# b-tudor/mpmcxx

Hardware: AMD Instinct MI355X
Metric: energy-evals/sec (10k-atom LJ+Ewald+polar box); 1/2/4/8-GPU scaling (higher is better)
Workload: dtype f64

## Files before the change

mpmcxx_amd/csrc/context.cpp:

```cpp
#include "context.h"

using namespace mpmc;

thread_local std::string mpmc::g_create_error;

extern "C" int mpmc_abi_version(void) { return MPMC_ABI_VERSION; }

extern "C" int mpmc_device_count(int *count) {
	int n = 0;
	hipError_t e = hipGetDeviceCount(&n);
	if (count) *count = (e == hipSuccess) ? n : 0;
	return (e == hipSuccess) ? MPMC_OK : MPMC_ERR_NO_DEVICE;
}

extern "C" int mpmc_device_synchronize(int device) {
	if (hipSetDevice(device) != hipSuccess) return MPMC_ERR_NO_DEVICE;
	return hipDeviceSynchronize() == hipSuccess ? MPMC_OK : MPMC_ERR_HIP;
}
extern "C" int mpmc_device_name(int device, char *name, int capacity) {
	if (!name || capacity < 1) return MPMC_ERR_ARG;
	name[0] = 0;
	hipDeviceProp_t prop;
	if (hipGetDeviceProperties(&prop, device) != hipSuccess) return MPMC_ERR_NO_DEVICE;
	std::snprintf(name, (size_t)capacity, "%s (%s, %d CUs)", prop.name, prop.gcnArchName, prop.multiProcessorCount);
// ... 1292 lines not shown
		if (v < -1 || v > 1) return MPMC_ERR_ARG;
		t.stream_mode = v;
	} else if (k == "pair_kernel") {
		if (v < 0 || v > 2) return MPMC_ERR_ARG;
		t.pair_kernel = v;
	} else if (k == "pair_waves") {
		if (v != 0 && v != 1 && v != 4) return MPMC_ERR_ARG;
		t.pair_waves = v;
	} else if (k == "fast_geometry") t.fast_geometry = on;
	else if (k == "dense_symmetric") t.dense_symmetric = on;
	else if (k == "sort_grid") {
		if (v < -1 || v > 0) return MPMC_ERR_ARG;
		t.sort_grid = v;
		if (c) c->atoms_dirty = c->atoms_dirty_order = true;
	} else if (k == "sort_nx") {
		t.sort_nx = v;
		if (c) c->atoms_dirty = c->atoms_dirty_order = true;
	} else if (k == "sort_ny") {
		t.sort_ny = v;
		if (c) c->atoms_dirty = c->atoms_dirty_order = true;
	}
	else if (k == "side_after_sweep") t.side_after_sweep = on;
	else if (k == "poll_long") t.poll_long = on;
	else if (k == "poll_retire") t.poll_retire = on;
	else if (k == "lazy_side_stream") t.lazy_side_stream = on;
	else if (k == "pair_split_tail") {
		if (v < -1 || v > 1000) return MPMC_ERR_ARG;
		t.pair_split_tail = v;
	} else if (k == "pair_split") {
		if (v < -1 || v > 1) return MPMC_ERR_ARG;
		t.pair_split = v;
	} else if (k == "panels") t.use_panels = on;
	else if (k == "sweep_order") {
		if (v < 0 || v > 1) return MPMC_ERR_ARG;
		t.sweep_order = v;
		if (c) c->sweep_tiles = -1, c->atoms_dirty = true;
	} else if (k == "sweep_lds_pad") {
		if (v < 0 || v > 65536) return MPMC_ERR_ARG;
		t.sweep_lds_pad = v;
	}
	else if (k == "uniform_images") t.no_uniform = !on;
	else if (k == "tile_classes") t.no_classes = !on;
	else if (k == "single_launch") t.single_launch = on;
	else if (k == "recip_table") t.no_recip_tab = !on;
	else if (k == "spatial_sort") {
		t.no_sort = !on;
		if (c) c->atoms_dirty = c->atoms_dirty_order = true;
	} else if (k == "order_carry") t.no_order_carry = !on;
	else if (k == "polar_delta") t.no_polar_delta = !on;
	else if (k == "inline_move") t.no_inline_move = !on;
	else if (k == "trace_panel") t.trace_panel = on;
	else if (k == "dipoles_on_demand") t.dipoles_on_demand = on;
	else if (k == "pef_phase_table") t.pef_phase_table = on;
	else if (k == "virtual_device") {
		if (!c || v < -1 || v > 63) return MPMC_ERR_ARG;
		t.virtual_device = v;
	} else if (k == "fail_next_wait") {
		if (!c) return MPMC_ERR_ARG;
		t.fail_next_wait = on ? 1 : 0;
	}
	else if (k == "panel_replicas") {
		if (!c || v < 1 || v > 64) return MPMC_ERR_ARG;
		c->debug_panel_replicas = v;
	} else if (k == "direct_budget_mb") {
		t.direct_budget_mb = (long long)value;
	} else if (k == "tensor_budget_mb") {
		if (value < 0) return MPMC_ERR_ARG;
		t.tensor_budget_mb = (long long)value;
	} else return MPMC_ERR_ARG;
	if (c && k != "panel_replicas" && k != "fail_next_wait" && k != "virtual_device" && k != "trace_panel") drop_pending_dipoles(c);
	return MPMC_OK;
}
extern "C" int mpmc_debug_last_trial_was_full(mpmc_ctx *c) { return (c && c->trial_last_kind >= 0) ? c->trial_last_kind : -1; }
extern "C" int mpmc_debug_last_pair_kernel(mpmc_ctx *c) { return c ? (c->last_pair_was_sweep ? 1 : 0) : -1; }

extern "C" int mpmc_debug_wait_counters(mpmc_ctx *c, long long *out4) {
	if (!c || !out4) return -1;
	out4[0] = c->kept.n_poll_hits;
	out4[1] = c->kept.n_poll_timeouts;
	out4[2] = c->kept.n_stream_syncs;
	out4[3] = c->kept.n_poll_yields;
	return 0;
}

extern "C" int mpmc_debug_upload_counts(mpmc_ctx *c, long long *out2) {
	if (!c || !out2) return -1;
	out2[0] = c->kept.n_uploads_carried;
	out2[1] = c->kept.n_uploads_sorted;
	return 0;
}

extern "C" int mpmc_debug_exchange_counts(mpmc_ctx *c, long long *out3) {
	if (!c || !out3) return -1;
	out3[0] = c->kept.n_xch_delta;
	out3[1] = c->kept.n_xch_full;
	out3[2] = c->kept.n_xch_resums;
	return 0;
}

extern "C" int mpmc_debug_panel_trace(mpmc_ctx *c, long long *out4, int max_entries) {
	if (!c || !out4) return -1;
	if (!c->d_trace) return 0;
	const int n = std::min(max_entries, c->n_panel_entries);
	if (hipSetDevice(c->device) != hipSuccess) return -1;
	if (hipMemcpyAsync(out4, c->d_trace, (size_t)n * 4 * sizeof(long long), hipMemcpyDeviceToHost, c->stream) != hipSuccess) return -1;
	if (hipStreamSynchronize(c->stream) != hipSuccess) return -1;
// ... 20 lines not shown
```

mpmcxx_amd/csrc/context.h:

```cpp
#pragma once
#include <hip/hip_runtime.h>

#include <algorithm>
#include <atomic>
#include <chrono>
#include <mutex>
#include <cmath>
#include <cstdio>
#include <cstdlib>
#include <cstring>
#include <string>
#include <thread>
#include <vector>

#include "../../include/mpmc_energy.h"
#include "kernels.h"

using namespace mpmc;

namespace mpmc {
extern thread_local std::string g_create_error;
}

struct EvPair {
// ... 19 lines not shown
	AnnotateHappensBefore(__FILE__, __LINE__, &g_pinned_pool_tag);
#endif
	return hipHostFree(p);
}

struct mpmc_ctx;
template <class T, bool kPinned = false>
struct DevBuf {
	T *p = nullptr;
	size_t cap = 0;
	DevBuf() = default;
	DevBuf(DevBuf &&o) noexcept : p(o.p), cap(o.cap) { o.p = nullptr, o.cap = 0; }
	DevBuf &operator=(DevBuf &&o) noexcept {
		std::swap(p, o.p), std::swap(cap, o.cap);
		return *this;
	}
	~DevBuf() { release(nullptr); }
	operator T *() const { return p; }
	void release(mpmc_ctx *c);
	int reserve(mpmc_ctx *c, size_t need, size_t grow_to = 0);
};
template <class T>
using PinnedBuf = DevBuf<T, true>;

struct mpmc_tuning {
	int stream_mode = -1;
	int pair_kernel = 0;
	int pair_waves = 0;
	int sort_grid = -1;
	int sort_nx = 0, sort_ny = 0;
	bool side_after_sweep = true;
	bool lazy_side_stream = true;
	bool poll_retire = true;
	bool poll_long = true;
	bool dense_symmetric = true;
	bool fast_geometry = true;
	int pair_split = -1;
	int pair_split_tail = -1;
	int sweep_order = 1;
	int sweep_lds_pad = 2048;
	bool use_panels = true;
	bool no_uniform = false;
	bool no_classes = false;
	bool single_launch = true;
	bool no_recip_tab = false;
	bool no_sort = false;
	bool no_order_carry = false;
	bool no_polar_delta = false;
	bool no_inline_move = false;
	int virtual_device = -1;
	int fail_next_wait = 0;
	bool trace_panel = false;
	bool dipoles_on_demand = true;
	bool pef_phase_table = true;
	long long tensor_budget_mb = 4096;
	long long direct_budget_mb = -1;
};

struct mpmc_kept {
	mpmc_tuning tune;
	bool prof = false;
	mpmc_timings tim{};
	long long n_poll_hits = 0, n_poll_timeouts = 0, n_stream_syncs = 0, n_poll_yields = 0;
	long long n_uploads_carried = 0, n_uploads_sorted = 0;
	long long n_xch_delta = 0, n_xch_full = 0, n_xch_resums = 0;
	bool tb_enabled = false, tb_mk = false;
	bool de_enabled = false;
	int de_flags = 0;
	bool pw_enabled = false;
	double pw_alpha = 0.0;
	bool palmo_enabled = false;
	bool rc_enabled = false;
	int rc_order = 0;
	int rdm_form = 0, rdm_mix = 0;
	bool pef_enabled = false;
	int pef_flags = 0;
	int relax_scheme = 0;
	bool zodid = false;
	bool on_demand = false;
	int cav_grid = 0;
	double cav_radius = 0.0;
};

struct AtomRun {
	std::vector<double> pos, q, alpha, eps, sigma, mass;
	std::vector<int32_t> mol, frozen, disp;
	int size() const { return (int)q.size(); }
	void clear() { pos.clear(), q.clear(), alpha.clear(), eps.clear(), sigma.clear(), mass.clear(), mol.clear(), frozen.clear(), disp.clear(); }
};
constexpr int kXchSums = 34, kXchClasses = 16, kXchResum = 1024;
struct XchSums {
	double s[kXchSums] = {0};
	long long cls[kXchClasses] = {0};
	int32_t mol_max = 0;
};

struct mpmc_ctx {
	mpmc_kept kept;
	int device = 0;
	hipStream_t stream = nullptr;
	hipStream_t stream2 = nullptr;
	hipEvent_t ev_fork = nullptr, ev_join = nullptr;
	bool two_streams = true;
	int max_atoms = 0, max_pad = 0;
	int n = 0, n_pad = 0, n_tiles = 0, n_tile_pairs = 0, n_split = 1;
	int n_molecules = 0;
// ... 35 lines not shown
	bool last_pair_was_sweep = false;
	FusedParams last_fp{};
	bool last_fp_valid = false;
	int debug_panel_replicas = 1;
	PinnedBuf<double4> h_xyzq;
	hipEvent_t ev_xyzq = nullptr;
	bool xyzq_in_flight = false;
	std::vector<double> h_pos_sorted;
	bool order_sorted = false;
	bool order_carried = false;
	bool atoms_dirty_order = false;
	int edits_since_sort = 0;
	double sort_origin_f[3] = {0, 0, 0};
	hipStream_t sync_stream = nullptr;
	std::vector<double> molmass_tmp;
	PinnedBuf<long long> static_cnt;
	PinnedBuf<char> h_kstage;
	hipEvent_t ev_kstage = nullptr;
	bool kstage_in_flight = false;
	int lvec_kmax = -1;
	PinnedBuf<char> h_stage;
	hipEvent_t ev_stage = nullptr;
	bool stage_in_flight = false;
	unsigned static_gen = 1, static_ride_gen = 0;

	bool static_dirty = true;
	double h_static[3] = {0, 0, 0};
	DevBuf<int> d_counter;
	bool scal_clean = false;
	int poll_budget_us = 1000;
	bool spin_on_post = false;
	bool last_was_single = false;
	double single_seq = 0;
	DevBuf<double> d_atom_part;
	DevBuf<double> d_scal;
	long long *d_cnt = nullptr;
	PinnedBuf<double> h_scal;
	long long *h_cnt = nullptr;
	DevBuf<int> d_flag;
	PinnedBuf<int> h_flag;

	int K = 0;
	DevBuf<double4> d_kvec, d_kw;
	DevBuf<double4> d_sf;
	DevBuf<int4> d_lvec;
	DevBuf<double4> d_sf_part;
	DevBuf<double> d_w_en;

	DevBuf<double> d_e_recip_part, d_part, d_e_static, d_mu[2], d_e_induced, d_rrms;
	DevBuf<double2> d_gs_blocks;
	DevBuf<double> d_gs_ul;
	int mu_cur = 0;
	DevBuf<double> d_dk_ring;
	enum { PEND_NONE = 0, PEND_OPEN = 1, PEND_DROPPED = 2 };
	int polar_pending = PEND_NONE;
	int pend_done = 0, pend_target = 0;
	DevBuf<double> d_arows;
	DevBuf<double> d_adense;
	DevBuf<double2> d_ab;
	int solver_used = MPMC_SOLVER_MATRIX_FREE;
	DevBuf<double> d_chol, d_chol_v, d_chol_info;
	PinnedBuf<double> h_chol_info;
	DevBuf<int> d_chol_list, d_chol_status;
	bool direct_ran = false;
	mpmc_direct_info direct{};

	Box box{};
	double box_in[20] = {0};
	bool box_in_has_recip = false;
	bool box_set = false, atoms_set = false, opts_set = false, k_dirty = true;
	mpmc_options opts{};
	double ewald_alpha = 0, polar_ewald_alpha = 0;

	bool pending = false;
	bool have_polar = false;
	int iters = 0, failed = 0;
	unsigned run_mask = 0;

	bool cache_valid = false;
	mpmc_result last_full{};
	mpmc_result trial_res{};
	int trial_last_kind = -1;
	bool trial_open = false, trial_evaluated = false, trial_was_full = false, trial_enqueued = false, trial_noop = false;
	mpmc_result trial_keep{};
	int trial_first = 0, trial_count = 0;
	std::vector<double> trial_new, trial_old;
	int *d_mv_slot = nullptr, *d_mv_orig = nullptr;
	double4 *d_mv_new = nullptr;
	DevBuf<int> d_moved_idx;
	DevBuf<double4> d_sf_trial;
	DevBuf<double> d_e_real, d_e_real_trial, d_dk_part;
	bool e_real_valid = false;
	bool trial_polar_delta = false;
	std::vector<int> store_dirty_tiles, trial_tiles;
	int touch_n = -1, touch[8] = {0};
	DevBuf<unsigned char> d_mv_blob;
	PinnedBuf<unsigned char> h_mv_blob;
	DevBuf<double> d_delta_out;
	PinnedBuf<double> h_delta_out;
	MvInline mv_inline{};
	bool trial_inline = false;
	double trial_seq = 0;
	long long *d_delta_cnt = nullptr, *h_delta_cnt = nullptr;

	int xch_kind = 0;
	int xch_at = 0;
// ... 204 lines not shown
	hipStream_t st;
	ProfScope(mpmc_ctx *c_, int cls, hipStream_t st_ = nullptr) : c(c_), st(st_ ? st_ : c_->stream) { prof_begin(c, cls, cur, st); }
	~ProfScope() { prof_end(c, cur, st); }
};
inline hipStream_t fork_side(mpmc_ctx *c) {
	if (!c->two_streams) return c->stream;
	if (!c->stream2 && hipStreamCreateWithFlags(&c->stream2, hipStreamNonBlocking) != hipSuccess) {
		c->stream2 = nullptr;
		c->two_streams = false;
		return c->stream;
	}
	(void)hipEventRecord(c->ev_fork, c->stream);
	(void)hipStreamWaitEvent(c->stream2, c->ev_fork, 0);
	return c->stream2;
}
inline void join_side(mpmc_ctx *c) {
	if (!c->two_streams || !c->stream2) return;
	(void)hipEventRecord(c->ev_join, c->stream2);
	(void)hipStreamWaitEvent(c->stream, c->ev_join, 0);
}


enum : unsigned {
	RUN_PAIR = 1, RUN_PAIR_ES = 2, RUN_RECIP = 4, RUN_ATOMTERMS = 8, RUN_FIELD = 16, RUN_SOLVE = 32, RUN_WOLF = 64,
	RUN_STORE = 128,
	RUN_THREE_BODY = 256,
	RUN_DISP = 512,
	RUN_CRYSTAL = 1024,
	RUN_RDM = 2048
};
constexpr double kThreeBodyScale = 3.0 * (0.0032539449 / (3.166811429 * 0.000001));
int three_body_ready(mpmc_ctx *c);
int disp_ready(mpmc_ctx *c);
DispParams disp_params(const mpmc_ctx *c);
inline bool rd_model_on(const mpmc_ctx *c) { return c->kept.rdm_form != 0 || c->kept.rdm_mix != 0; }
inline bool crystal_on(const mpmc_ctx *c) { return c->kept.rc_enabled && !c->kept.de_enabled && c->kept.rdm_form == 0; }
int rd_model_ready(mpmc_ctx *c);
RdModelParams rd_model_params(const mpmc_ctx *c);
int crystal_ready(mpmc_ctx *c);
CrystalParams crystal_params(const mpmc_ctx *c);
Box lrc_box(const mpmc_ctx *c);
int prepare(mpmc_ctx *c, bool defer_static = false);
int enqueue(mpmc_ctx *c, unsigned mask, bool on_demand = false);
int wait_and_fill(mpmc_ctx *c, mpmc_result *out);
unsigned full_mask(const mpmc_ctx *c);
inline bool polar_moments_apply(const mpmc_ctx *c) {
	const mpmc_options &o = c->opts;
	if (c->kept.relax_scheme != 0 || c->kept.zodid) return false;
	if (c->kept.pef_enabled) return false;
	return o.polarization && !o.rd_only && o.polar_iterative && o.polar_max_iter >= 1 && o.polar_max_iter <= kMomentsMaxIter && o.polar_gamma == 1.0 && o.polar_precision == 0.0 && !o.polar_rrms &&
	       !o.polar_gs;
}
inline int moments_half(int n) { return (n + 1) / 2; }
inline int reserve_dk_ring(mpmc_ctx *c) { return c->d_dk_ring.reserve(c, (size_t)(moments_half(c->opts.polar_max_iter) + 1) * 3 * (size_t)c->max_pad); }
int finish_pending_dipoles(mpmc_ctx *c);
inline bool ewald_full_on(const mpmc_ctx *c) { return c->kept.pef_enabled && c->opts.polarization && !c->opts.rd_only; }
inline bool field_is_ewald(const mpmc_ctx *c) { return c->opts.polar_ewald || ewald_full_on(c); }
inline void drop_pending_dipoles(mpmc_ctx *c) {
	if (c->polar_pending == mpmc_ctx::PEND_OPEN) c->polar_pending = mpmc_ctx::PEND_DROPPED;
}
inline bool direct_solve(const mpmc_ctx *c) {
	return c->opts.polarization && !c->opts.rd_only && !c->opts.polar_iterative && !ewald_full_on(c);
}
inline bool zodid_on(const mpmc_ctx *c) {
	return c->kept.zodid && c->opts.polarization && !c->opts.rd_only && c->opts.polar_iterative && !ewald_full_on(c);
}
inline double start_gamma(const mpmc_ctx *c) { return (ewald_full_on(c) || c->kept.relax_scheme != 0) ? 1.0 : c->opts.polar_gamma; }
inline bool wolf_field_on(const mpmc_ctx *c) { return c->kept.pw_enabled && c->opts.polarization && !c->opts.rd_only && !field_is_ewald(c); }
void ext_params(const mpmc_ctx *c, FusedParams &fp, bool wolf_on);
AtomsDev atoms_view(const mpmc_ctx *c);
RecipDev recip_view(const mpmc_ctx *c);
int upload_atoms(mpmc_ctx *c);
inline int atom_flag_word(const mpmc_ctx *c, int frozen, double eps, double sigma, int disp, double q, double alpha) {
	int fl = 0;
	if (frozen) fl |= AF_FROZEN;
	if (eps == 0.0 || sigma == 0.0) fl |= AF_NULL_RD;
	if (disp) fl |= c->kept.de_enabled ? AF_DISP_RD : AF_HAS_DISP;
	if (sigma < 0.0) fl |= AF_NEG_SIGMA;
	if (sigma == 0.0) fl |= AF_ZERO_SIGMA;
	if (q == 0.0) fl |= AF_ZERO_Q;
	if (alpha == 0.0) fl |= AF_ZERO_ALPHA;
	return fl;
}
int splice_atoms(mpmc_ctx *c, int at, int n_remove, const AtomRun *ins);
void copy_atom_run(const mpmc_ctx *c, int first, int count, AtomRun &out);
int set_atoms_from(mpmc_ctx *c, const AtomRun &list);
void xch_sum_list(const mpmc_ctx *c, XchSums &out);
void xch_sum_atom(const mpmc_ctx *c, XchSums &xs, double sg, int fl, double sigma, double eps, double q);
void xch_static_terms(const mpmc_ctx *c, const XchSums &xs, double out3[3]);
void wrap_molecules(const mpmc_ctx *c, double *com, double *wrapped_com, double *wrapped_pos);

}
```

mpmcxx_amd/csrc/evaluate.cpp:

```cpp
#include "context.h"


using namespace mpmc;

static int build_k_tables(mpmc_ctx *c) {
	const int kmax = c->opts.ewald_kmax;
	const double alpha = c->ewald_alpha, ea = c->polar_ewald_alpha;
	auto each_lvec = [kmax](auto &&visit) {
		int l[3];
		for (l[0] = 0; l[0] <= kmax; l[0]++)
			for (l[1] = (!l[0] ? 0 : -kmax); l[1] <= kmax; l[1]++)
				for (l[2] = ((!l[0] && !l[1]) ? 1 : -kmax); l[2] <= kmax; l[2]++)
					if (l[0] * l[0] + l[1] * l[1] + l[2] * l[2] <= kmax * kmax) visit(l);
	};
	int K = 0, rc;
	each_lvec([&K](const int *) { K++; });
	if ((size_t)K > c->d_lvec.cap) c->lvec_kmax = -1;
	if ((rc = c->d_kvec.reserve(c, (size_t)K)) != MPMC_OK) return rc;
	if ((rc = c->d_kw.reserve(c, (size_t)K)) != MPMC_OK) return rc;
	if ((rc = c->d_lvec.reserve(c, (size_t)K)) != MPMC_OK) return rc;
	if ((rc = c->d_w_en.reserve(c, (size_t)K)) != MPMC_OK) return rc;
	if ((rc = c->d_sf.reserve(c, (size_t)K)) != MPMC_OK) return rc;
	if (K > 0) {
		if (c->kstage_in_flight) {
// ... 738 lines not shown
	int passes = 0;
	for (bool keep = true; keep;) {
		if (passes >= kMaxIterationCount && p.by_precision) {
			c->failed = 1;
			break;
		}
		if (p.by_precision) HIP_TRY(c, hipMemsetAsync(c->d_flag, 0, sizeof(int), st));
		{
			ProfScope ps(c, MPMC_K_DIPOLE_ITER);
			launch_pef_contract(st, at, c->box, c->d_mu[c->mu_cur], c->d_tile_pairs, c->n_tile_pairs, c->d_pef_cnt, c->d_pef_store, c->d_part);
			launch_pef_sf(st, at, rcp.kvec, c->K, phases, c->d_mu[c->mu_cur], c->d_pef_psum);
		}
		{
			ProfScope ps(c, MPMC_K_REDUCE);
			const RelaxWeights rw = relax_weights(p.relax, o.polar_gamma, passes + 1);
			launch_pef_finish(st, at, ep, c->d_e_static, c->d_part, c->n_tiles, phases, rcp.kvec, rcp.kw, c->K, c->d_pef_psum, c->d_mu[c->mu_cur],
			                  c->d_mu[1 - c->mu_cur], c->d_e_induced, p.by_precision ? c->d_flag.p : nullptr, p.relax ? &rw : nullptr);
		}
		c->mu_cur = 1 - c->mu_cur;
		if (p.by_precision) {
			HIP_TRY(c, hipMemcpyAsync(c->h_flag, c->d_flag, sizeof(int), hipMemcpyDeviceToHost, st));
			HIP_TRY(c, hipStreamSynchronize(st));
			keep = (*c->h_flag != 0);
		} else {
			keep = (passes != o.polar_max_iter);
		}
		passes++;
	}
	HIP_TRY(c, hipGetLastError());
	c->iters = 0;
	c->polar_pending = mpmc_ctx::PEND_NONE;
	c->pef_ran = true;
	c->pef_info.passes = passes;
	c->pef_info.n_k = c->K;
	c->pef_info.store_bytes = (int64_t)(c->d_pef_store.cap * sizeof(double2));
	c->relax_info.acted = (p.relax != RELAX_NONE && passes > 0) ? 1 : 0;
	c->relax_info.contractions = passes;
	c->relax_info.last_weight = relax_weights(p.relax, o.polar_gamma, passes).w_new;
	c->relax_info.store_filled = 1;
	return MPMC_OK;
}

static int stage_polar_energy(mpmc_ctx *c, const EvalPlan &p, const AtomsDev &at, const RecipDev &) {
	if (!p.solve) return MPMC_OK;
	hipStream_t st = c->stream;
	if (p.zodid) {
		c->mu_cur = 0;
		HIP_TRY(c, hipMemsetAsync(c->d_e_induced, 0, 3 * (size_t)at.n_pad * sizeof(double), st));
		c->polar_pending = mpmc_ctx::PEND_NONE;
		c->relax_info.acted = 1;
	}
	const double *mu = c->d_mu[c->mu_cur], *rrms = p.want_rrms ? c->d_rrms.p : nullptr;
	ProfScope ps(c, MPMC_K_REDUCE);
	if (p.moments && p.reduce_in_tail)
		launch_polar_moments_and_pairs(st, at, c->d_dk_ring, c->d_e_static, c->opts.polar_max_iter, c->d_block_part, c->d_block_cnt, c->n_tile_pairs, c->d_scal,
		                               c->d_cnt);
	else if (p.moments) launch_polar_moments(st, at, c->d_dk_ring, c->d_e_static, c->opts.polar_max_iter, c->d_scal);
	else if (p.reduce_in_tail)
		launch_polar_energy_and_pairs(st, at, mu, c->d_e_static, rrms, c->d_block_part, c->d_block_cnt, c->n_tile_pairs, c->d_scal, c->d_cnt);
	else launch_polar_energy(st, at, mu, c->d_e_static, rrms, c->d_scal);
	c->have_polar = true;
	return MPMC_OK;
}

static int stage_palmo(mpmc_ctx *c, const EvalPlan &p, const AtomsDev &at, const RecipDev &) {
	if (!p.palmo || c->failed) return MPMC_OK;
	double *mu = c->d_mu[c->mu_cur];
	double *contracted = p.relax ? c->d_mu[1 - c->mu_cur].p : mu, *spare = p.relax ? c->d_palmo_change.p : c->d_mu[1 - c->mu_cur].p;
	contract_into_field(c, at, contracted, spare, c->d_palmo_f, true,
	                    [&] { launch_palmo_reduce(c->stream, at, mu, c->d_palmo_f, c->d_e_induced, c->d_palmo_change, c->d_scal); });
	c->palmo_ran = true;
	c->relax_info.contractions += 1;
	return MPMC_OK;
}

static int stage_added_terms(mpmc_ctx *c, const EvalPlan &p, const AtomsDev &at, const RecipDev &) {
	hipStream_t st = c->stream;
	if (p.mask & RUN_THREE_BODY) {
		ProfScope ps(c, MPMC_K_THREE_BODY);
		launch_three_body(st, at, c->d_tb_au, c->box, kThreeBodyScale, c->d_tb_part, c->d_scal + S_THREE_BODY);
	}
	if (p.mask & RUN_DISP) {
		ProfScope ps(c, MPMC_K_PAIR);
		launch_disp_expansion(st, at, c->d_de_co, c->d_de_t10, c->d_tile_pairs, c->n_tile_pairs, c->box, disp_params(c), c->de_lrc[0], c->de_lrc[1],
		                      c->d_de_part, c->d_scal + S_DISP);
	}
	if (p.mask & RUN_CRYSTAL) {
		ProfScope ps(c, MPMC_K_PAIR);
		launch_crystal(st, at, c->box, crystal_params(c), c->d_rc_shift, c->d_tile_pairs, c->n_tile_pairs, c->d_rc_part, c->d_scal + S_CRYSTAL);
	}
	if (p.mask & RUN_RDM) {
		ProfScope ps(c, MPMC_K_PAIR);
		const int *cls = (p.pair_pass && c->box.ortho && !c->kept.tune.no_classes) ? c->d_cls.p : nullptr;
		launch_rd_model(st, at, c->d_rdm_sp, c->d_tile_pairs, cls, c->n_tile_pairs, c->box, rd_model_params(c), c->d_rdm_part, c->d_scal + S_RDM);
	}
	HIP_TRY(c, hipGetLastError());
	return MPMC_OK;
}

static int stage_post(mpmc_ctx *c, const EvalPlan &, const AtomsDev &, const RecipDev &) {
	c->single_seq += 1.0;
	launch_post_results(c->stream, c->d_scal, c->h_scal, c->single_seq);
	HIP_TRY(c, hipGetLastError());
	c->scal_clean = true;
	c->spin_on_post = c->ev_used.empty() && (c->kept.tune.poll_long || c->n_tile_pairs <= kOneStreamMaxPairs);
	c->poll_budget_us = (c->n_tile_pairs <= kOneStreamMaxPairs) ? 1000 : 4000;
	c->pending = true;
	return MPMC_OK;
}

// ... 460 lines not shown
```

mpmcxx_amd/csrc/kernels.h:

```cpp
#pragma once

#include <hip/hip_runtime.h>
#include <stdint.h>

#include <algorithm>
#include <type_traits>

#include "pair_math.h"
#include "polar_relax.h"

namespace mpmc {

template <class F>
inline void with_flag(bool a, F &&f) {
	if (a) f(std::true_type{});
	else f(std::false_type{});
}
template <class F>
inline void with_flags(bool a, bool b, F &&f) {
	with_flag(a, [&](auto A) { with_flag(b, [&](auto B) { f(A, B); }); });
}

constexpr int kTile = 64;
constexpr int kKSplit = 8;
// ... 30 lines not shown
enum : int { C_LJ_IN = 0, C_ES_IN, C_INTRA, C_RDX, C_ESX, C_FROZEN, C_COUNT = 8 };
enum : int {
	D_LJ = 0, D_ES_REAL, D_ES_INTRA, D_ES_RECIP, D_SPARE,
	D_CNT_LJ, D_CNT_ES,
	D_THREE_BODY,
	D_DISP,
	D_RD, D_RD_TERMS,
	D_COUNT
};
static_assert(D_RD_TERMS == D_RD + 1, "the delta launchers of the rd terms write { sum, terms } side by side");
constexpr int kDeltaHostSeq = D_THREE_BODY + 1;
constexpr int kDeltaHostCount = D_COUNT + 1;
constexpr int delta_host_index(int d) { return d < kDeltaHostSeq ? d : d + 1; }
enum : int {
	CLS_BEYOND_CUTOFF = 1,
	CLS_THOLE_FAR = 2,
	CLS_UNIFORM_X = 4,
	CLS_UNIFORM_Y = 8,
	CLS_UNIFORM_Z = 16
};
constexpr double kTholeFarX = 30.0;

struct RecipDev {
	const double4 *kvec;
	const double *w_en;
	const double4 *kw;
	const int4 *lvec;
	double4 *sf;
	int K;
};
constexpr int kRecipTabMaxK = 15;
void launch_recip_sf(hipStream_t st, const AtomsDev &at, const Box &bx, const RecipDev &rc, int kmax, double4 *sf_part);
constexpr size_t kAtomTermScratch = 64 * 34;
void launch_atom_terms(hipStream_t st, const AtomsDev &at, const Box &bx, double ewald_alpha, int rd_lrc, int do_es, double *part_scratch,
                       double *scal);

void launch_field_recip(hipStream_t st, const AtomsDev &at, const Box &bx, const RecipDev &rc, int kmax, double *e_recip );
void launch_field_finalize(hipStream_t st, const AtomsDev &at, const Box &bx, int polar_ewald, const double *e_recip,
                           const double *part, int n_split, double gamma, double *e_static, double *mu,
                           double *e_real_out = nullptr ,
                           double *mu_copy = nullptr );

void launch_dipole_update(hipStream_t st, const AtomsDev &at, const double *e_static, const double *part, int n_split,
                          const double *mu_old, double *mu_new, double *e_induced, int want_rrms, double *rrms_atom,
                          double allowed_sqerr, int *ctl, int *host_flag , int it,
                          double *dk = nullptr ,
                          const RelaxWeights *relax = nullptr );
void launch_dipole_reset(hipStream_t st, const AtomsDev &at, const double *e_static, double *mu);
void launch_post_results(hipStream_t st, double *scal, double *out_host, double seq);
void launch_polar_energy(hipStream_t st, const AtomsDev &at, const double *mu, const double *e_static, const double *rrms_atom,
                         double *scal);
constexpr int kMomentsMaxIter = 64;
constexpr int kMomentsMaxHalf = (kMomentsMaxIter + 1) / 2;
void launch_polar_moments(hipStream_t st, const AtomsDev &at, const double *dk, const double *e_static, int n_iter, double *scal);
void launch_polar_moments_and_pairs(hipStream_t st, const AtomsDev &at, const double *dk, const double *e_static, int n_iter,
                                    const double *block_part, const int *block_cnt, int nb, double *scal, long long *cnt);

void launch_amatrix_rows(hipStream_t st, const AtomsDev &at, const int *slot_of, const Box &bx, double polar_damp, int row0, int nrows,
                         double *a );

struct FusedParams {
	double ewald_alpha, polar_ewald_alpha, polar_damp;
	int rd_lrc;
	int do_es;
	int do_field;
	int do_thole;
	int wolf;
	int fh_order;
	double fh_c2, fh_c4;
	double wolf_erfa_over_r, wolf_inv_r2;
	double thole_far_x;
	int store_only;
	int touch_n;
	int touch[8];
	int pair_waves;
};
constexpr int kOneStreamMaxPairs = 1536;
constexpr int kPairSplitMax = 8192;
void launch_pair_fused(hipStream_t st, const AtomsDev &at, const Box &bx, const FusedParams &fp, const int2 *tile_pairs,
                       const int *cls, int n_tile_pairs, double *block_part , int *block_cnt , double *fpart, double2 *ab,
                       const int *tp_list = nullptr);
struct PairSweepParams {
	double alpha_scaled_half, polar_damp_half, thole_far_x;
	int store;
	int nt;
	int have_shift;
	int split;
	int n_main;
	int fast;
};
constexpr int kSweepMinPairs = 2048;
constexpr int kSweepSplitTailPermille = 250;
constexpr int kErfTableDouble2 = 3 * 512;
void erfc_table_device_layout(double2 *out );
int pair_sweep_blocks(int n_tiles, int2 *out);
bool pair_sweep_covers(const Box &bx, const FusedParams &fp, double ewald_alpha);
void launch_pair_sweep(hipStream_t st, const AtomsDev &at, const Box &bx, const FusedParams &fp, bool intra ,
                       const int2 *blocks, int n_blocks, const int *cls, const double4 *tp_shift ,
                       const double2 *erf_tab, double *block_part, int *block_cnt, double *fpart, double2 *ab, int split_mode = 0 ,
                       int n_split_tail = 0 , bool fast_geometry = false, int lds_pad_bytes = 0 ,
                       int replicas = 1 );
void launch_reduce_pairs(hipStream_t st, const double *block_part, const int *block_cnt, int nb, double *scal, long long *cnt);
void launch_polar_energy_and_pairs(hipStream_t st, const AtomsDev &at, const double *mu, const double *e_static, const double *rrms_atom,
                                   const double *block_part, const int *block_cnt, int nb, double *scal, long long *cnt);
void launch_pair_lj_single(hipStream_t st, const AtomsDev &at, const Box &bx, const FusedParams &fp, const int2 *tile_pairs, int n_tile_pairs,
                           double *block_part, int *block_cnt, int *counter, double *out_host, double seq);
void launch_recip_energy(hipStream_t st, const RecipDev &rc, const Box &bx, double *scal);
void launch_static_counts(hipStream_t st, const AtomsDev &at, const int2 *tile_pairs, int n_tile_pairs, int *block_cnt ,
// ... 172 lines not shown
```

mpmcxx_amd/csrc/kernels.hip:

```cpp
#include "kernels.h"
#include "device_math.h"

namespace mpmc {

__device__ __forceinline__ void reduce_pairs_block(const double *__restrict__ block_part, const int *__restrict__ block_cnt, int nb,
                                                   double *__restrict__ scal, long long *__restrict__ cnt) {
	__shared__ double sh[4];
	__shared__ long long shc[256];
	double s0 = 0, s1 = 0;
	long long c0 = 0, c1 = 0;
#pragma unroll 4
	for (int b = threadIdx.x; b < nb; b += 256) {
		s0 += block_part[2 * (size_t)b];
		s1 += block_part[2 * (size_t)b + 1];
		c0 += block_cnt[2 * (size_t)b];
		c1 += block_cnt[2 * (size_t)b + 1];
	}
	s0 = block_sum_256(s0, sh);
	s1 = block_sum_256(s1, sh);
	if (threadIdx.x == 0) {
		scal[S_LJ] = s0;
		scal[S_ES_REAL] = s1;
	}
	c0 = block_count_256(c0, shc);
// ... 501 lines not shown
		if (!isfinite(r)) r = 0.0;
		rrms_atom[i] = (i < at.n) ? r : 0.0;
	}
	if (ctl) iteration_verdict(ctl, host_flag, it, allowed_sqerr > 0.0 && broke && i < at.n);
}
__global__ __launch_bounds__(512) void k_dipole_update(AtomsDev at, const double *__restrict__ e_static, const double *__restrict__ part,
                                                       int n_split, const double *__restrict__ mu_old, double *__restrict__ mu_new,
                                                       double *__restrict__ e_induced, int want_rrms, double *__restrict__ rrms_atom,
                                                       double allowed_sqerr, int *__restrict__ ctl, int *__restrict__ host_flag, int it,
                                                       double *__restrict__ dk) {
	dipole_update_block<false>(at, e_static, part, n_split, mu_old, mu_new, e_induced, want_rrms, rrms_atom, allowed_sqerr, ctl, host_flag, it, dk);
}
__global__ __launch_bounds__(512) void k_dipole_update_relax(AtomsDev at, const double *__restrict__ e_static, const double *__restrict__ part,
                                                             int n_split, const double *__restrict__ mu_old, double *__restrict__ mu_new,
                                                             double *__restrict__ e_induced, int want_rrms, double *__restrict__ rrms_atom,
                                                             double allowed_sqerr, int *__restrict__ ctl, int *__restrict__ host_flag, int it,
                                                             double *__restrict__ dk, RelaxWeights w) {
	dipole_update_block<true>(at, e_static, part, n_split, mu_old, mu_new, e_induced, want_rrms, rrms_atom, allowed_sqerr, ctl, host_flag, it, dk,
	                          w.w_new, w.w_old);
}

__global__ __launch_bounds__(256) void k_dipole_reset(AtomsDev at, const double *__restrict__ e_static, double *__restrict__ mu) {
	const int i = blockIdx.x * 256 + threadIdx.x;
	if (i >= at.n_pad) return;
	const double a = at.alpha[i];
	for (int p = 0; p < 3; ++p) mu[3 * (size_t)i + p] = a * e_static[3 * (size_t)i + p];
}

__device__ __forceinline__ void polar_energy_block(const AtomsDev &at, const double *__restrict__ mu, const double *__restrict__ e_static,
                                                   const double *__restrict__ rrms_atom, double *__restrict__ scal) {
	__shared__ double sh[4];
	double u = 0, rr = 0;
#pragma unroll 4
	for (int i = threadIdx.x; i < at.n; i += 256) {
		const size_t b = 3 * (size_t)i;
		u += ((mu[b] * e_static[b]) + mu[b + 1] * e_static[b + 1]) + mu[b + 2] * e_static[b + 2];
		if (rrms_atom) {
			const double r = rrms_atom[i];
			if (isfinite(r)) rr += r;
		}
	}
	u = block_sum_256(u, sh);
	rr = block_sum_256(rr, sh);
	if (threadIdx.x == 0) {
		scal[S_POLAR] = -0.5 * u;
		scal[S_RRMS] = rr / (double)at.n;
	}
}
__global__ __launch_bounds__(256) void k_polar_energy(AtomsDev at, const double *__restrict__ mu, const double *__restrict__ e_static,
                                                      const double *__restrict__ rrms_atom, double *__restrict__ scal) {
	polar_energy_block(at, mu, e_static, rrms_atom, scal);
}

constexpr int kMomentsMax = 2 * (kMomentsMaxHalf + 1);
constexpr int kMomentsOnePassHalf = 5;
template <int H>
__device__ __forceinline__ void polar_moments_one_pass(const AtomsDev &at, const double *__restrict__ dk, const double *__restrict__ e_static,
                                                       double *__restrict__ sh, double *__restrict__ s_m) {
	const size_t stride = 3 * (size_t)at.n_pad;
	double acc[2 * H + 1] = {};
#pragma unroll 2
	for (int i = threadIdx.x; i < at.n; i += 256) {
		const size_t b = 3 * (size_t)i;
		const double al = at.alpha[i];
		double d[H + 1][3], w[3];
#pragma unroll
		for (int a = 0; a <= H; ++a) {
			const double *__restrict__ q = dk + (size_t)a * stride + b;
			d[a][0] = q[0], d[a][1] = q[1], d[a][2] = q[2];
		}
		w[0] = e_static[b], w[1] = e_static[b + 1], w[2] = e_static[b + 2];
		const double inv = (al != 0.0) ? 1.0 / al : 0.0;
#pragma unroll
		for (int a = 0; a <= H; ++a) {
			if (a > 0) w[0] = d[a][0] * inv, w[1] = d[a][1] * inv, w[2] = d[a][2] * inv;
			acc[2 * a] += ((w[0] * d[a][0]) + w[1] * d[a][1]) + w[2] * d[a][2];
			if (a < H) acc[2 * a + 1] += ((w[0] * d[a + 1][0]) + w[1] * d[a + 1][1]) + w[2] * d[a + 1][2];
		}
	}
#pragma unroll
	for (int k = 0; k <= 2 * H; ++k) {
		const double v = block_sum_256(acc[k], sh);
		if (threadIdx.x == 0) s_m[k] = v;
	}
}
__device__ __forceinline__ void polar_moments_block(const AtomsDev &at, const double *__restrict__ dk, const double *__restrict__ e_static, int n_iter,
                                                    double *__restrict__ scal) {
	__shared__ double sh[4];
	__shared__ double s_m[kMomentsMax];
	const size_t stride = 3 * (size_t)at.n_pad;
	const int half = (n_iter + 1) / 2;
	switch (half <= kMomentsOnePassHalf ? half : 0) {
	case 1: polar_moments_one_pass<1>(at, dk, e_static, sh, s_m); break;
	case 2: polar_moments_one_pass<2>(at, dk, e_static, sh, s_m); break;
	case 3: polar_moments_one_pass<3>(at, dk, e_static, sh, s_m); break;
	case 4: polar_moments_one_pass<4>(at, dk, e_static, sh, s_m); break;
	case 5: polar_moments_one_pass<5>(at, dk, e_static, sh, s_m); break;
	default: break;
	}
	for (int a = 0; a <= (half <= kMomentsOnePassHalf ? -1 : half); ++a) {
		const double *__restrict__ da = dk + (size_t)a * stride;
		const bool odd = 2 * a + 1 <= n_iter;
		const double *__restrict__ db = odd ? da + stride : da;
		double m0 = 0, m1 = 0;
		if (a == 0) {
#pragma unroll 4
			for (int i = threadIdx.x; i < at.n; i += 256) {
				const size_t b = 3 * (size_t)i;
				const double w0 = e_static[b], w1 = e_static[b + 1], w2 = e_static[b + 2];
				m0 += ((w0 * da[b]) + w1 * da[b + 1]) + w2 * da[b + 2];
				m1 += ((w0 * db[b]) + w1 * db[b + 1]) + w2 * db[b + 2];
			}
		} else {
#pragma unroll 4
			for (int i = threadIdx.x; i < at.n; i += 256) {
				const size_t b = 3 * (size_t)i;
				const double al = at.alpha[i];
				const double inv = (al != 0.0) ? 1.0 / al : 0.0;
				const double w0 = da[b] * inv, w1 = da[b + 1] * inv, w2 = da[b + 2] * inv;
				m0 += ((w0 * da[b]) + w1 * da[b + 1]) + w2 * da[b + 2];
				m1 += ((w0 * db[b]) + w1 * db[b + 1]) + w2 * db[b + 2];
			}
		}
		m0 = block_sum_256(m0, sh);
		m1 = block_sum_256(m1, sh);
		if (threadIdx.x == 0) {
			s_m[2 * a] = m0;
			s_m[2 * a + 1] = odd ? m1 : 0.0;
		}
	}
	if (threadIdx.x == 0) {
		double u = 0;
		for (int k = 0; k <= n_iter; ++k) u += s_m[k];
		scal[S_POLAR] = -0.5 * u;
		scal[S_RRMS] = 0.0;
	}
}
__global__ __launch_bounds__(256) void k_polar_moments(AtomsDev at, const double *__restrict__ dk, const double *__restrict__ e_static, int n_iter,
                                                       double *__restrict__ scal) {
	polar_moments_block(at, dk, e_static, n_iter, scal);
}
__global__ __launch_bounds__(256) void k_polar_moments_and_pairs(AtomsDev at, const double *__restrict__ dk, const double *__restrict__ e_static, int n_iter,
                                                                 const double *__restrict__ block_part, const int *__restrict__ block_cnt, int nb,
                                                                 double *__restrict__ scal, long long *__restrict__ cnt) {
	if (blockIdx.x == 0) polar_moments_block(at, dk, e_static, n_iter, scal);
	else reduce_pairs_block(block_part, block_cnt, nb, scal, cnt);
}
void launch_polar_moments(hipStream_t st, const AtomsDev &at, const double *dk, const double *e_static, int n_iter, double *scal) {
	hipLaunchKernelGGL(k_polar_moments, dim3(1), dim3(256), 0, st, at, dk, e_static, n_iter, scal);
}
void launch_polar_moments_and_pairs(hipStream_t st, const AtomsDev &at, const double *dk, const double *e_static, int n_iter, const double *block_part,
                                    const int *block_cnt, int nb, double *scal, long long *cnt) {
	hipLaunchKernelGGL(k_polar_moments_and_pairs, dim3(2), dim3(256), 0, st, at, dk, e_static, n_iter, block_part, block_cnt, nb, scal, cnt);
}

__global__ __launch_bounds__(256) void k_polar_energy_and_pairs(AtomsDev at, const double *__restrict__ mu, const double *__restrict__ e_static,
                                                                const double *__restrict__ rrms_atom, const double *__restrict__ block_part,
                                                                const int *__restrict__ block_cnt, int nb, double *__restrict__ scal,
                                                                long long *__restrict__ cnt) {
	if (blockIdx.x == 0) polar_energy_block(at, mu, e_static, rrms_atom, scal);
	else reduce_pairs_block(block_part, block_cnt, nb, scal, cnt);
}

void launch_dipole_update(hipStream_t st, const AtomsDev &at, const double *e_static, const double *part, int n_split, const double *mu_old,
                          double *mu_new, double *e_induced, int want_rrms, double *rrms_atom, double allowed_sqerr, int *ctl, int *host_flag, int it,
                          double *dk, const RelaxWeights *relax) {
	if (relax)
		hipLaunchKernelGGL(k_dipole_update_relax, dim3(at.n_pad / kTile), dim3(kTile * kSlotGroups), 0, st, at, e_static, part, n_split, mu_old, mu_new,
		                   e_induced, want_rrms, rrms_atom, allowed_sqerr, ctl, host_flag, it, dk, *relax);
	else
		hipLaunchKernelGGL(k_dipole_update, dim3(at.n_pad / kTile), dim3(kTile * kSlotGroups), 0, st, at, e_static, part, n_split, mu_old, mu_new,
		                   e_induced, want_rrms, rrms_atom, allowed_sqerr, ctl, host_flag, it, dk);
}
void launch_dipole_reset(hipStream_t st, const AtomsDev &at, const double *e_static, double *mu) {
	hipLaunchKernelGGL(k_dipole_reset, dim3((at.n_pad + 255) / 256), dim3(256), 0, st, at, e_static, mu);
}
void launch_polar_energy(hipStream_t st, const AtomsDev &at, const double *mu, const double *e_static, const double *rrms_atom, double *scal) {
	hipLaunchKernelGGL(k_polar_energy, dim3(1), dim3(256), 0, st, at, mu, e_static, rrms_atom, scal);
}
void launch_polar_energy_and_pairs(hipStream_t st, const AtomsDev &at, const double *mu, const double *e_static, const double *rrms_atom,
                                   const double *block_part, const int *block_cnt, int nb, double *scal, long long *cnt) {
	hipLaunchKernelGGL(k_polar_energy_and_pairs, dim3(2), dim3(256), 0, st, at, mu, e_static, rrms_atom, block_part, block_cnt, nb, scal, cnt);
}

template <bool ORTHO>
__global__ __launch_bounds__(256) void k_amatrix_rows(AtomsDev at, const int *__restrict__ slot_of, Box bx, double lambda, int atom0,
                                                      int natoms_rows, double *__restrict__ a) {
	const int j = blockIdx.x * 256 + threadIdx.x;
	const int ir = blockIdx.y;
	if (j >= at.n || ir >= natoms_rows) return;
	const int i = atom0 + ir;
	const size_t ld = 3 * (size_t)at.n;
	double *blk = a + (3 * (size_t)ir) * ld + 3 * (size_t)j;
	if (i == j) {
		const double al = at.alpha[slot_of[i]];
		for (int p = 0; p < 3; ++p)
			for (int q = 0; q < 3; ++q) blk[p * ld + q] = (p == q) ? ((al != 0.0) ? 1.0 / al : kMaxValue) : 0.0;
		return;
	}
	const int lo = min(i, j), hi = max(i, j);
	const double4 pl = at.xyzq[slot_of[lo]], ph = at.xyzq[slot_of[hi]];
	double d[3];
	const double r = min_image<ORTHO>(bx, pl.x - ph.x, pl.y - ph.y, pl.z - ph.z, d[0], d[1], d[2]);
	double ir3, ir5;
	if (r == 0.0)
		ir3 = ir5 = kMaxValue;
// ... 42 lines not shown
```

Baseline: 1945.

## Split polar moment reduction into multi-block partials kernel plus fold

Replaces the single-block polar moments reduction, which used a fused one-pass template for small iteration counts, with a two-stage scheme. A grid of 64-thread blocks, one column per moment pair, writes per-virtual-thread partials to a device buffer, and the existing single block then folds them. This spreads the dot-product work over many CUs instead of one, at the cost of an extra kernel launch and a partials buffer. The old one-pass path that read each dk array once is removed, so dk and e_static may be re-read per moment pair.

```diff
diff --git a/mpmcxx_amd/csrc/context.cpp b/mpmcxx_amd/csrc/context.cpp
--- a/mpmcxx_amd/csrc/context.cpp
+++ b/mpmcxx_amd/csrc/context.cpp
@@ -1368,6 +1368,7 @@
 	else if (k == "trace_panel") t.trace_panel = on;
 	else if (k == "dipoles_on_demand") t.dipoles_on_demand = on;
 	else if (k == "pef_phase_table") t.pef_phase_table = on;
+	else if (k == "moments_one_block") t.moments_one_block = on;
 	else if (k == "virtual_device") {
 		if (!c || v < -1 || v > 63) return MPMC_ERR_ARG;
 		t.virtual_device = v;
diff --git a/mpmcxx_amd/csrc/context.h b/mpmcxx_amd/csrc/context.h
--- a/mpmcxx_amd/csrc/context.h
+++ b/mpmcxx_amd/csrc/context.h
@@ -95,6 +95,7 @@
 	int fail_next_wait = 0;
 	bool trace_panel = false;
 	bool dipoles_on_demand = true;
+	bool moments_one_block = false;
 	bool pef_phase_table = true;
 	long long tensor_budget_mb = 4096;
 	long long direct_budget_mb = -1;
@@ -236,6 +237,7 @@
 	DevBuf<double> d_gs_ul;
 	int mu_cur = 0;
 	DevBuf<double> d_dk_ring;
+	DevBuf<double> d_moment_part;
 	enum { PEND_NONE = 0, PEND_OPEN = 1, PEND_DROPPED = 2 };
 	int polar_pending = PEND_NONE;
 	int pend_done = 0, pend_target = 0;
@@ -546,7 +548,10 @@
 	       !o.polar_gs;
 }
 inline int moments_half(int n) { return (n + 1) / 2; }
-inline int reserve_dk_ring(mpmc_ctx *c) { return c->d_dk_ring.reserve(c, (size_t)(moments_half(c->opts.polar_max_iter) + 1) * 3 * (size_t)c->max_pad); }
+inline int reserve_dk_ring(mpmc_ctx *c) {
+	const int rc = c->d_dk_ring.reserve(c, (size_t)(moments_half(c->opts.polar_max_iter) + 1) * 3 * (size_t)c->max_pad);
+	return rc != MPMC_OK ? rc : c->d_moment_part.reserve(c, kMomentPartials);
+}
 int finish_pending_dipoles(mpmc_ctx *c);
 inline bool ewald_full_on(const mpmc_ctx *c) { return c->kept.pef_enabled && c->opts.polarization && !c->opts.rd_only; }
 inline bool field_is_ewald(const mpmc_ctx *c) { return c->opts.polar_ewald || ewald_full_on(c); }
diff --git a/mpmcxx_amd/csrc/evaluate.cpp b/mpmcxx_amd/csrc/evaluate.cpp
--- a/mpmcxx_amd/csrc/evaluate.cpp
+++ b/mpmcxx_amd/csrc/evaluate.cpp
@@ -814,10 +814,11 @@
 	}
 	const double *mu = c->d_mu[c->mu_cur], *rrms = p.want_rrms ? c->d_rrms.p : nullptr;
 	ProfScope ps(c, MPMC_K_REDUCE);
+	double *moment_part = c->kept.tune.moments_one_block ? nullptr : c->d_moment_part.p;
 	if (p.moments && p.reduce_in_tail)
-		launch_polar_moments_and_pairs(st, at, c->d_dk_ring, c->d_e_static, c->opts.polar_max_iter, c->d_block_part, c->d_block_cnt, c->n_tile_pairs, c->d_scal,
-		                               c->d_cnt);
-	else if (p.moments) launch_polar_moments(st, at, c->d_dk_ring, c->d_e_static, c->opts.polar_max_iter, c->d_scal);
+		launch_polar_moments_and_pairs(st, at, c->d_dk_ring, c->d_e_static, c->opts.polar_max_iter, moment_part, c->d_block_part, c->d_block_cnt, c->n_tile_pairs,
+		                               c->d_scal, c->d_cnt);
+	else if (p.moments) launch_polar_moments(st, at, c->d_dk_ring, c->d_e_static, c->opts.polar_max_iter, moment_part, c->d_scal);
 	else if (p.reduce_in_tail)
 		launch_polar_energy_and_pairs(st, at, mu, c->d_e_static, rrms, c->d_block_part, c->d_block_cnt, c->n_tile_pairs, c->d_scal, c->d_cnt);
 	else launch_polar_energy(st, at, mu, c->d_e_static, rrms, c->d_scal);
diff --git a/mpmcxx_amd/csrc/kernels.h b/mpmcxx_amd/csrc/kernels.h
--- a/mpmcxx_amd/csrc/kernels.h
+++ b/mpmcxx_amd/csrc/kernels.h
@@ -106,8 +106,11 @@
                          double *scal);
 constexpr int kMomentsMaxIter = 64;
 constexpr int kMomentsMaxHalf = (kMomentsMaxIter + 1) / 2;
-void launch_polar_moments(hipStream_t st, const AtomsDev &at, const double *dk, const double *e_static, int n_iter, double *scal);
-void launch_polar_moments_and_pairs(hipStream_t st, const AtomsDev &at, const double *dk, const double *e_static, int n_iter,
+constexpr int kMomentsMax = 2 * (kMomentsMaxHalf + 1);
+constexpr int kMomentThreads = 256;
+constexpr size_t kMomentPartials = (size_t)kMomentsMax * kMomentThreads;
+void launch_polar_moments(hipStream_t st, const AtomsDev &at, const double *dk, const double *e_static, int n_iter, double *partial, double *scal);
+void launch_polar_moments_and_pairs(hipStream_t st, const AtomsDev &at, const double *dk, const double *e_static, int n_iter, double *partial,
                                     const double *block_part, const int *block_cnt, int nb, double *scal, long long *cnt);
 
 void launch_amatrix_rows(hipStream_t st, const AtomsDev &at, const int *slot_of, const Box &bx, double polar_damp, int row0, int nrows,
diff --git a/mpmcxx_amd/csrc/kernels.hip b/mpmcxx_amd/csrc/kernels.hip
--- a/mpmcxx_amd/csrc/kernels.hip
+++ b/mpmcxx_amd/csrc/kernels.hip
@@ -577,84 +577,74 @@
 	polar_energy_block(at, mu, e_static, rrms_atom, scal);
 }
 
-constexpr int kMomentsMax = 2 * (kMomentsMaxHalf + 1);
-constexpr int kMomentsOnePassHalf = 5;
-template <int H>
-__device__ __forceinline__ void polar_moments_one_pass(const AtomsDev &at, const double *__restrict__ dk, const double *__restrict__ e_static,
-                                                       double *__restrict__ sh, double *__restrict__ s_m) {
+__device__ __forceinline__ void polar_moment_pair(const AtomsDev &at, const double *__restrict__ dk, const double *__restrict__ e_static, int n_iter, int a,
+                                                  int t, double &m0_out, double &m1_out) {
 	const size_t stride = 3 * (size_t)at.n_pad;
-	double acc[2 * H + 1] = {};
-#pragma unroll 2
-	for (int i = threadIdx.x; i < at.n; i += 256) {
-		const size_t b = 3 * (size_t)i;
-		const double al = at.alpha[i];
-		double d[H + 1][3], w[3];
-#pragma unroll
-		for (int a = 0; a <= H; ++a) {
-			const double *__restrict__ q = dk + (size_t)a * stride + b;
-			d[a][0] = q[0], d[a][1] = q[1], d[a][2] = q[2];
-		}
-		w[0] = e_static[b], w[1] = e_static[b + 1], w[2] = e_static[b + 2];
-		const double inv = (al != 0.0) ? 1.0 / al : 0.0;
-#pragma unroll
-		for (int a = 0; a <= H; ++a) {
-			if (a > 0) w[0] = d[a][0] * inv, w[1] = d[a][1] * inv, w[2] = d[a][2] * inv;
-			acc[2 * a] += ((w[0] * d[a][0]) + w[1] * d[a][1]) + w[2] * d[a][2];
-			if (a < H) acc[2 * a + 1] += ((w[0] * d[a + 1][0]) + w[1] * d[a + 1][1]) + w[2] * d[a + 1][2];
-		}
-	}
-#pragma unroll
-	for (int k = 0; k <= 2 * H; ++k) {
-		const double v = block_sum_256(acc[k], sh);
-		if (threadIdx.x == 0) s_m[k] = v;
-	}
+	const double *__restrict__ da = dk + (size_t)a * stride;
+	const bool odd = 2 * a + 1 <= n_iter;
+	const double *__restrict__ db = odd ? da + stride : da;
+	double m0 = 0, m1 = 0;
+	if (a == 0) {
+#pragma unroll 4
+		for (int i = t; i < at.n; i += kMomentThreads) {
+			const size_t b = 3 * (size_t)i;
+			const double w0 = e_static[b], w1 = e_static[b + 1], w2 = e_static[b + 2];
+			m0 += ((w0 * da[b]) + w1 * da[b + 1]) + w2 * da[b + 2];
+			m1 += ((w0 * db[b]) + w1 * db[b + 1]) + w2 * db[b + 2];
+		}
+	} else {
+#pragma unroll 4
+		for (int i = t; i < at.n; i += kMomentThreads) {
+			const size_t b = 3 * (size_t)i;
+			const double al = at.alpha[i];
+			const double inv = (al != 0.0) ? 1.0 / al : 0.0;
+			const double w0 = da[b] * inv, w1 = da[b + 1] * inv, w2 = da[b + 2] * inv;
+			m0 += ((w0 * da[b]) + w1 * da[b + 1]) + w2 * da[b + 2];
+			m1 += ((w0 * db[b]) + w1 * db[b + 1]) + w2 * db[b + 2];
+		}
+	}
+	m0_out = m0;
+	m1_out = odd ? m1 : 0.0;
+}
+__global__ __launch_bounds__(64) void k_polar_moment_partials(AtomsDev at, const double *__restrict__ dk, const double *__restrict__ e_static, int n_iter,
+                                                              double *__restrict__ partial) {
+	const int a = blockIdx.y, t = blockIdx.x * 64 + threadIdx.x;
+	double m0, m1;
+	polar_moment_pair(at, dk, e_static, n_iter, a, t, m0, m1);
+	partial[(size_t)(2 * a) * kMomentThreads + t] = m0;
+	partial[(size_t)(2 * a + 1) * kMomentThreads + t] = m1;
 }
 __device__ __forceinline__ void polar_moments_block(const AtomsDev &at, const double *__restrict__ dk, const double *__restrict__ e_static, int n_iter,
-                                                    double *__restrict__ scal) {
+                                                    const double *__restrict__ partial, double *__restrict__ scal) {
 	__shared__ double sh[4];
 	__shared__ double s_m[kMomentsMax];
-	const size_t stride = 3 * (size_t)at.n_pad;
-	const int half = (n_iter + 1) / 2;
-	switch (half <= kMomentsOnePassHalf ? half : 0) {
-	case 1: polar_moments_one_pass<1>(at, dk, e_static, sh, s_m); break;
-	case 2: polar_moments_one_pass<2>(at, dk, e_static, sh, s_m); break;
-	case 3: polar_moments_one_pass<3>(at, dk, e_static, sh, s_m); break;
-	case 4: polar_moments_one_pass<4>(at, dk, e_static, sh, s_m); break;
-	case 5: polar_moments_one_pass<5>(at, dk, e_static, sh, s_m); break;
-	default: break;
-	}
-	for (int a = 0; a <= (half <= kMomentsOnePassHalf ? -1 : half); ++a) {
-		const double *__restrict__ da = dk + (size_t)a * stride;
-		const bool odd = 2 * a + 1 <= n_iter;
-		const double *__restrict__ db = odd ? da + stride : da;
-		double m0 = 0, m1 = 0;
-		if (a == 0) {
-#pragma unroll 4
-			for (int i = threadIdx.x; i < at.n; i += 256) {
-				const size_t b = 3 * (size_t)i;
-				const double w0 = e_static[b], w1 = e_static[b + 1], w2 = e_static[b + 2];
-				m0 += ((w0 * da[b]) + w1 * da[b + 1]) + w2 * da[b + 2];
-				m1 += ((w0 * db[b]) + w1 * db[b + 1]) + w2 * db[b + 2];
+	static_assert(kMomentThreads == 256, "one virtual thread per thread of the folding block");
+	const int t = threadIdx.x;
+	if (partial) {
+		for (int k0 = 0; k0 <= n_iter; k0 += 4) {
+			double v[4];
+#pragma unroll
+			for (int j = 0; j < 4; ++j) v[j] = partial[(size_t)min(k0 + j, n_iter) * kMomentThreads + t];
+#pragma unroll
+			for (int j = 0; j < 4; ++j) {
+				if (k0 + j > n_iter) break;
+				const double m = block_sum_256(v[j], sh);
+				if (t == 0) s_m[k0 + j] = m;
 			}
-		} else {
-#pragma unroll 4
-			for (int i = threadIdx.x; i < at.n; i += 256) {
-				const size_t b = 3 * (size_t)i;
-				const double al = at.alpha[i];
-				const double inv = (al != 0.0) ? 1.0 / al : 0.0;
-				const double w0 = da[b] * inv, w1 = da[b + 1] * inv, w2 = da[b + 2] * inv;
-				m0 += ((w0 * da[b]) + w1 * da[b + 1]) + w2 * da[b + 2];
-				m1 += ((w0 * db[b]) + w1 * db[b + 1]) + w2 * db[b + 2];
+		}
+	} else {
+		for (int a = 0; 2 * a <= n_iter; ++a) {
+			double m0, m1;
+			polar_moment_pair(at, dk, e_static, n_iter, a, t, m0, m1);
+			m0 = block_sum_256(m0, sh);
+			m1 = block_sum_256(m1, sh);
+			if (t == 0) {
+				s_m[2 * a] = m0;
+				s_m[2 * a + 1] = m1;
 			}
 		}
-		m0 = block_sum_256(m0, sh);
-		m1 = block_sum_256(m1, sh);
-		if (threadIdx.x == 0) {
-			s_m[2 * a] = m0;
-			s_m[2 * a + 1] = odd ? m1 : 0.0;
-		}
-	}
-	if (threadIdx.x == 0) {
+	}
+	if (t == 0) {
 		double u = 0;
 		for (int k = 0; k <= n_iter; ++k) u += s_m[k];
 		scal[S_POLAR] = -0.5 * u;
@@ -662,21 +652,26 @@
 	}
 }
 __global__ __launch_bounds__(256) void k_polar_moments(AtomsDev at, const double *__restrict__ dk, const double *__restrict__ e_static, int n_iter,
-                                                       double *__restrict__ scal) {
-	polar_moments_block(at, dk, e_static, n_iter, scal);
+                                                       const double *__restrict__ partial, double *__restrict__ scal) {
+	polar_moments_block(at, dk, e_static, n_iter, partial, scal);
 }
 __global__ __launch_bounds__(256) void k_polar_moments_and_pairs(AtomsDev at, const double *__restrict__ dk, const double *__restrict__ e_static, int n_iter,
-                                                                 const double *__restrict__ block_part, const int *__restrict__ block_cnt, int nb,
-                                                                 double *__restrict__ scal, long long *__restrict__ cnt) {
-	if (blockIdx.x == 0) polar_moments_block(at, dk, e_static, n_iter, scal);
+                                                                 const double *__restrict__ partial, const double *__restrict__ block_part,
+                                                                 const int *__restrict__ block_cnt, int nb, double *__restrict__ scal, long long *__restrict__ cnt) {
+	if (blockIdx.x == 0) polar_moments_block(at, dk, e_static, n_iter, partial, scal);
 	else reduce_pairs_block(block_part, block_cnt, nb, scal, cnt);
 }
-void launch_polar_moments(hipStream_t st, const AtomsDev &at, const double *dk, const double *e_static, int n_iter, double *scal) {
-	hipLaunchKernelGGL(k_polar_moments, dim3(1), dim3(256), 0, st, at, dk, e_static, n_iter, scal);
-}
-void launch_polar_moments_and_pairs(hipStream_t st, const AtomsDev &at, const double *dk, const double *e_static, int n_iter, const double *block_part,
-                                    const int *block_cnt, int nb, double *scal, long long *cnt) {
-	hipLaunchKernelGGL(k_polar_moments_and_pairs, dim3(2), dim3(256), 0, st, at, dk, e_static, n_iter, block_part, block_cnt, nb, scal, cnt);
+static void launch_polar_moment_partials(hipStream_t st, const AtomsDev &at, const double *dk, const double *e_static, int n_iter, double *partial) {
+	hipLaunchKernelGGL(k_polar_moment_partials, dim3(kMomentThreads / 64, n_iter / 2 + 1), dim3(64), 0, st, at, dk, e_static, n_iter, partial);
+}
+void launch_polar_moments(hipStream_t st, const AtomsDev &at, const double *dk, const double *e_static, int n_iter, double *partial, double *scal) {
+	if (partial) launch_polar_moment_partials(st, at, dk, e_static, n_iter, partial);
+	hipLaunchKernelGGL(k_polar_moments, dim3(1), dim3(256), 0, st, at, dk, e_static, n_iter, partial, scal);
+}
+void launch_polar_moments_and_pairs(hipStream_t st, const AtomsDev &at, const double *dk, const double *e_static, int n_iter, double *partial,
+                                    const double *block_part, const int *block_cnt, int nb, double *scal, long long *cnt) {
+	if (partial) launch_polar_moment_partials(st, at, dk, e_static, n_iter, partial);
+	hipLaunchKernelGGL(k_polar_moments_and_pairs, dim3(2), dim3(256), 0, st, at, dk, e_static, n_iter, partial, block_part, block_cnt, nb, scal, cnt);
 }
 
 __global__ __launch_bounds__(256) void k_polar_energy_and_pairs(AtomsDev at, const double *__restrict__ mu, const double *__restrict__ e_static,
```

New measurement: 1944, median of 3. Within noise of the previous version (-0.0%).
